# falcon-computing/falcon-genome

Hardware: AMD Instinct MI355X
Metric: PairHMM GCUPS + banded-SW GCUPS per GPU; end-to-end htc regions/sec at 8 GPUs (higher is better)
Workload: dtype fp32 (fp64 rescue)

## Files before the change

### falcon-genome_amd/csrc/phmm_cols.h

```cpp
#pragma once

namespace fcs {

constexpr int kColsClasses = 8;
constexpr int kColsMinR = 33;
__host__ __device__ constexpr int cols_C(int c) { return c == 0 ? 19 : 18 - c; }
__host__ __device__ constexpr int cols_hmax(int c) { return 16 * cols_C(c) - 1; }
__host__ __device__ inline int cols_class(int H) {
  for (int c = kColsClasses - 1; c >= 0; --c)
    if (H <= cols_hmax(c)) return c;
  return -1;
}
constexpr int kColsRing = 32;
constexpr int kColsChunks = 6;
constexpr int kColsChunkBytes = kColsRing * 4 * 16;
constexpr int kColsCapOff = kColsChunks * kColsChunkBytes;
constexpr int kColsTabOff = kColsCapOff + 4 * 8 * 8;
constexpr int kColsLds = kColsTabOff + 3 * 128 * 4;

__device__ __forceinline__ uint32_t vconst(uint32_t k) {
  uint32_t r;
  asm volatile("v_mov_b32 %0, %1" : "=v"(r) : "i"(k));
  return r;
}

struct ColsItem {
  float e1, e3, my, yy, mm, gm, mx, xx;
  uint32_t tlo, thi;
  float z;
};

__device__ __forceinline__ ColsItem cols_item(const PhmmTables<float>& tab, const RawRow& raw, int role, bool first,
                                              float ih) {
  ColsItem c;
  if (role == 2 || role == 3) {
    const RowP<float> q = row_params<float, false>(tab, raw);
    const float x0 = first ? ih * tab.dmatch[raw.gq & 127] : 1.f;
    const bool last = role == 3;
    c.e1 = q.e1 * x0;
    c.e3 = q.e3 * x0;
    c.my = last ? 0.f : q.my;
    c.yy = q.yy;
    c.mm = last ? 1.f : q.mm;
    c.gm = last ? 1.f : q.gm;
    c.mx = last ? 0.f : q.mx;
    c.xx = last ? 0.f : q.xx;
    const int bc = base_code((unsigned char)raw.rb);
    c.tlo = bc < 4 ? 1u << (8 * bc) : bc == 4 ? vconst(0x01010101u) : 0u;
    c.thi = 0x00000001u;
    c.z = 0.f;
  } else if (role == 4) {
    c.e1 = 1.f;
    c.e3 = 0.f;
    c.my = c.yy = c.mm = c.gm = 1.f;
    c.mx = c.xx = 0.f;
    c.tlo = vconst(0x01010101u);
    c.thi = vconst(0x00000101u);
    c.z = 0.f;
  } else {
    c.e1 = c.e3 = c.my = c.mm = c.gm = c.mx = c.xx = 0.f;
    c.yy = 1.f;
    c.tlo = c.thi = 0u;
    c.z = 1.f;
  }
  return c;
}

__device__ __forceinline__ void cols_put(unsigned char* smem, int slot, int seg, int h, const ColsItem& c) {
  float* const p = reinterpret_cast<float*>(smem + (seg * kColsRing + slot) * 16) + h;
  constexpr int F = kColsChunkBytes / 4;
  p[0] = c.e1;
  p[2] = c.e3;
  p[F] = c.my;
  p[F + 2] = c.yy;
  p[2 * F] = c.mm;
  p[2 * F + 2] = c.gm;
  p[3 * F] = c.mx;
  p[3 * F + 2] = c.xx;
  uint32_t* const q = reinterpret_cast<uint32_t*>(p);
  q[4 * F] = c.tlo;
  q[4 * F + 2] = c.thi;
  q[5 * F] = __float_as_uint(c.z);
  q[5 * F + 2] = __float_as_uint(c.z);
}

template <int NW>
__device__ __forceinline__ void cols_convert(const uint32_t (&raw)[NW + 1], int al, int i0, int H, uint32_t (&code)[NW],
                                             bool& other) {
#pragma unroll
  for (int d = 0; d < NW; ++d) {
    const uint32_t x = __builtin_amdgcn_alignbyte(raw[d + 1], raw[d], (uint32_t)al);
    const int rel = H - (i0 + 4 * d);
    const int nv = min(max(rel, 0), 4);
    const uint32_t vmask = nv >= 4 ? 0xFFFFFFFFu : (1u << (8 * nv)) - 1u;
    const uint32_t sel = (x >> 1) & vconst(0x07070707u);
    uint32_t c = __builtin_amdgcn_perm(vconst(0x04050505u), vconst(0x02030100u), sel);
    const uint32_t back = __builtin_amdgcn_perm(vconst(0x0000004Eu), vconst(0x54474341u), c);
    other |= ((back ^ x) & vmask) != 0u;
    c = (c & vmask) | (vconst(0x06060606u) & ~vmask);
    if (rel >= 0 && rel < 4) c = (c & ~(0xFFu << (8 * rel))) | (0x05u << (8 * rel));
    code[d] = c;
  }
}

template <int NW>
__device__ __forceinline__ void cols_load(const uint8_t* __restrict__ hb, int64_t ho, int H, int i0, uint32_t (&raw)[NW + 1],
                                          int& al) {
  const int64_t s = ho + i0;
  al = (int)(s & 3);
  const int64_t base = s - al;
  const uint32_t* const src = reinterpret_cast<const uint32_t*>(hb + base);
#pragma unroll
  for (int d = 0; d <= NW; ++d) raw[d] = (base + 4 * d < ho + H && H > 0) ? src[d] : 0u;
}

template <int C>
__global__ __launch_bounds__(64, 2) void phmm4_kernel(
    const PhmmDevBatch b, const int32_t* __restrict__ order, const int64_t* __restrict__ bounds, const int cls,
    const int K, const int tail_pairs, const PhmmTables<float> gtab, double* __restrict__ out,
    int32_t* __restrict__ rescue_list, unsigned long long* __restrict__ rescue_count, const float thr,
    const int use_rescue, int32_t* __restrict__ fb_list, unsigned long long* __restrict__ fb_count) {
  constexpr int NW = (C + 3) / 4;
  extern __shared__ __align__(16) unsigned char smem_raw[];
  const int lane = threadIdx.x;
  const int seg = lane >> 4;
  const int sl = lane & 15;
  const int sbase = lane & 48;
  const int th = sl >> 3, tk = sl & 7;
  const int i0 = sl * C;
  const int64_t cbeg = bounds[cls];
  const long long count = bounds[cls + 1] - cbeg;
  order += cbeg;
  PhmmTables<float> tab = gtab;
  {
    float* const t = reinterpret_cast<float*>(smem_raw + kColsTabOff);
    for (int i = lane; i < 128; i += 64) {
      t[i] = gtab.ph2pr[i];
      t[128 + i] = gtab.dmatch[i];
      t[256 + i] = gtab.dmis[i];
    }
    tab.ph2pr = t;
    tab.dmatch = t + 128;
    tab.dmis = t + 256;
  }
  const long long tailn = count < (long long)tail_pairs ? count : (long long)tail_pairs;
  const long long headn = count - tailn;
  const long long per = 8LL * K;
  const long long nb_head = (headn + per - 1) / per;
  const long long nbatch = nb_head + (tailn + 7) / 8;

  for (long long w = blockIdx.x; w < nbatch; w += gridDim.x) {
    const bool head = w < nb_head;
    const int Kb = head ? K : 1;
    const long long bstart = head ? w * per : headn + (w - nb_head) * 8;
    const long long bend = head ? min(headn, bstart + per) : min(count, bstart + 8);
    const long long idx = bstart + 2 * seg + th + 8LL * tk;
    const int pm = (tk < Kb && idx < bend) ? order[idx] : -1;
    int Rm = 0, Hm = 0;
    int64_t rom = 0, hom = 0;
    float Im = 0.f;
    if (pm >= 0) {
      const int ri = b.pair_read[pm], hi = b.pair_hap[pm];
      Rm = b.read_len[ri];
      Hm = b.hap_len[hi];
      rom = b.read_off[ri];
      hom = b.hap_off[hi];
      Im = tab.init_const / (float)Hm;
    }
    const int len = pm >= 0 ? Rm + 2 : 0;
    int incl = len;
#pragma unroll
    for (int d = 1; d < 8; d <<= 1) {
      const int v = __shfl_up(incl, d, 8);
      if (tk >= d) incl += v;
    }
    const int Gm = incl - len;
    const int totA = __builtin_amdgcn_ds_bpermute(4 * (sbase + 7), incl);
    const int totB = __builtin_amdgcn_ds_bpermute(4 * (sbase + 15), incl);
    const int nsteps = ((wave_max(max(totA, totB)) + 15) + 7) & ~7;
    int sb = sbase * 4;
    auto bp = [&](int v, int h, int k) {
      return __builtin_amdgcn_ds_bpermute(sb + 4 * (8 * h + min(k, 7)), v);
    };
    auto tG = [&](int h, int k) { return bp(Gm, h, k); };
    auto tR = [&](int h, int k) { return bp(Rm, h, k); };
    auto tH = [&](int h, int k) { return bp(Hm, h, k); };
    auto tP = [&](int h, int k) { return bp(pm, h, k); };
    auto tI = [&](int h, int k) { return __int_as_float(bp(__float_as_int(Im), h, k)); };
    auto t64 = [&](int64_t v, int h, int k) {
      const int lo = bp((int)v, h, k), hi = bp((int)(v >> 32), h, k);
      return (int64_t)(((uint64_t)(uint32_t)hi << 32) | (uint32_t)lo);
    };
    auto valid = [&](int h, int k) {
      const int pv = tP(h, k);
      return k < Kb && pv >= 0;
    };

    uint32_t cur[2][NW], nxt[2][NW];
    int nk[2], swr[2];
    unsigned other[2] = {0u, 0u};
    auto fetch_codes = [&](int h, int k, uint32_t (&dst)[NW]) {
      const bool ok = valid(h, k);
      const int Hk = tH(h, k);
      const int H = ok ? Hk : 0;
      const int64_t ho = t64(hom, h, k);
      uint32_t raw[NW + 1];
      int al;
      cols_load<NW>(b.hb, ok ? ho : 0, H, i0, raw, al);
      bool oth = false;
      cols_convert<NW>(raw, al, i0, H, dst, oth);
      const unsigned long long bal = __ballot(oth && ok);
      if (((bal >> sbase) & 0xFFFFull) != 0ull) other[h] |= 1u << k;
    };
#pragma unroll
    for (int h = 0; h < 2; ++h) {
#pragma unroll
      for (int d = 0; d < NW; ++d) cur[h][d] = 0x06060606u;
      fetch_codes(h, 0, nxt[h]);
      nk[h] = 0;
      swr[h] = valid(h, 0) ? tG(h, 0) : 0x3FFFFFFF;
    }
    int kc[2] = {0, 0};
    int cap[2], capp[2];
    auto load_cap = [&](int h) {
      const bool ok = valid(h, kc[h]);
      const int v = tG(h, kc[h]) + tR(h, kc[h]);
      cap[h] = ok ? v : -0x3FFFFFFF;
      capp[h] = tP(h, kc[h]);
    };
    load_cap(0);
    load_cap(1);

    int kp = 0;
    RawRow praw{-1, 0, 0, 0, 0, 0, 0};
    int prole = 0;
    float pih = 0.f;
    bool kok = false, nok = false;
    int kG = 0, kR = 0, nG = 0;
    float kI = 0.f;
    int64_t kro = 0;
    auto load_cursor = [&] {
      kok = valid(th, kp);
      kG = tG(th, kp);
      kR = tR(th, kp);
      kI = tI(th, kp);
      kro = t64(rom, th, kp);
      nok = valid(th, kp + 1);
      nG = tG(th, kp + 1);
    };
    load_cursor();
    auto stage_a = [&](int base) {
      const int g = base + tk;
      const bool adv = nok && g >= nG;
      if (__ballot(adv) != 0ull) {
        if (adv) ++kp;
        load_cursor();
      }
      const bool ok = kok;
      const int G = kG, R = kR;
      pih = kI;
      const int64_t ro = kro;
      const int r = g - G;
      int role = 0;
      if (ok && r >= 0 && r < R) role = r == R - 1 ? 3 : 2;
      else if (ok && r == R) role = 4;
      prole = role | (r == 0 ? 16 : 0);
      praw = (role == 2 || role == 3) ? load_raw(b, R, ro, r) : RawRow{-1, 0, 0, 0, 0, 0, 0};
    };
    auto stage_b = [&](int base) {
      cols_put(smem_raw, (base + tk) & (kColsRing - 1), seg, th,
               cols_item(tab, praw, prole & 15, (prole & 16) != 0, pih));
    };
    {
      ColsItem z = cols_item(tab, RawRow{-1, 0, 0, 0, 0, 0, 0}, 0, false, 0.f);
      cols_put(smem_raw, 16 + tk, seg, th, z);
      cols_put(smem_raw, 24 + tk, seg, th, z);
      stage_a(0);
      stage_b(0);
      stage_a(8);
    }

    pf2 Xn[C], In[C];
#pragma unroll
    for (int j = 0; j < C; ++j) {
      Xn[j] = pf2{1.f, 1.f};
      In[j] = pf2{0.f, 0.f};
    }
    pf2 dn = pf2{1.f, 1.f}, xo = pf2{1.f, 1.f}, xin = pf2{1.f, 1.f};
    const uint32_t segoff = (uint32_t)seg * (kColsRing * 16u) + lds_addr(smem_raw);

    for (int t0 = 0; t0 < nsteps; t0 += 8) {
      asm volatile("" : "+v"(sb));
#pragma unroll
      for (int h = 0; h < 2; ++h) {
        const bool ev = swr[h] + 16 <= t0 && nk[h] + 1 < Kb;
        if (__ballot(ev) != 0ull) {
          uint32_t tmp[NW];
          fetch_codes(h, nk[h] + 1, tmp);
          const bool vn = valid(h, nk[h] + 1);
          const int gn = tG(h, nk[h] + 1);
          if (ev) {
#pragma unroll
            for (int d = 0; d < NW; ++d) nxt[h][d] = tmp[d];
            ++nk[h];
            swr[h] = vn ? gn : 0x3FFFFFFF;
          }
        }
        if (swr[h] + 16 <= t0 && nk[h] + 1 >= Kb) swr[h] = 0x3FFFFFFF;
      }
      stage_b(t0 + 8);
      stage_a(t0 + 16);
#pragma unroll
      for (int h = 0; h < 2; ++h) {
        const bool adv = cap[h] >= 0 && cap[h] + 15 < t0;
        if (__ballot(adv) != 0ull) {
          if (adv) ++kc[h];
          load_cap(h);
        }
      }
      bool capo[2];
#pragma unroll
      for (int h = 0; h < 2; ++h) capo[h] = (other[h] >> kc[h]) & 1u;
      const int g0 = t0 - sl;
      const bool any_cap = __ballot(sl == 15 && ((unsigned)(cap[0] - g0) < 8u || (unsigned)(cap[1] - g0) < 8u)) != 0ull;
      unsigned swmask = 0u;
#pragma unroll
      for (int q = 0; q < 4; ++q)
#pragma unroll
        for (int h = 0; h < 2; ++h) {
          const int lo = __builtin_amdgcn_readlane(swr[h], 16 * q) - t0;
          if (lo < 8 && lo + 15 >= 0) {
            const int a = max(lo, 0), bnd = min(lo + 15, 7);
            swmask |= ((2u << bnd) - 1u) & ~((1u << a) - 1u);
          }
        }
      const uint32_t xs = (uint32_t)(g0 & (kColsRing - 1)) * 16u;
      const uint32_t capa = lds_addr(smem_raw) + kColsCapOff + seg * 64;

      auto step = [&](auto S_) {
        constexpr int S = decltype(S_)::value;
        const int g = g0 + S;
        if (swmask & (1u << S)) {
#pragma unroll
          for (int h = 0; h < 2; ++h) {
            const bool take = g == swr[h];
#pragma unroll
            for (int d = 0; d < NW; ++d) {
              uint32_t r;
              asm("v_cndmask_b32_e64 %0, %1, %2, %3" : "=v"(r) : "v"(cur[h][d]), "v"(nxt[h][d]), "s"(__ballot(take)));
              cur[h][d] = r;
            }
          }
        }
        asm volatile("" ::: "memory");
        const uint32_t pa = ((xs + (uint32_t)(S * 16)) & (uint32_t)((kColsRing - 1) * 16)) + segoff;
        typedef float f4 __attribute__((ext_vector_type(4)));
        typedef uint32_t u4 __attribute__((ext_vector_type(4)));
        auto ld4 = [&](int chunk) {
          return *reinterpret_cast<const __attribute__((address_space(3))) f4*>((uintptr_t)(pa + chunk * kColsChunkBytes));
        };
        const f4 r0 = ld4(0), r1 = ld4(1), r2 = ld4(2), r3 = ld4(3);
        const u4 cr = *reinterpret_cast<const __attribute__((address_space(3))) u4*>((uintptr_t)(pa + 4 * kColsChunkBytes));
        const pf2 z1 = *reinterpret_cast<const __attribute__((address_space(3))) pf2*>((uintptr_t)(pa + 5 * kColsChunkBytes));
        const pf2 z2 = *reinterpret_cast<const __attribute__((address_space(3))) pf2*>((uintptr_t)(pa + 5 * kColsChunkBytes + 8));
        const pf2 e1 = pf2{r0.x, r0.y}, e3 = pf2{r0.z, r0.w}, my = pf2{r1.x, r1.y}, yy = pf2{r1.z, r1.w};
        const pf2 mm = pf2{r2.x, r2.y}, gm = pf2{r2.z, r2.w}, mx = pf2{r3.x, r3.y}, xx = pf2{r3.z, r3.w};
        pf2 din, xnx;
        din.x = __int_as_float(__builtin_amdgcn_update_dpp(__float_as_int(z1.x), __float_as_int(dn.x), kDppRowShr1, 0xF, 0xF, false));
        din.y = __int_as_float(__builtin_amdgcn_update_dpp(__float_as_int(z1.y), __float_as_int(dn.y), kDppRowShr1, 0xF, 0xF, false));
        xnx.x = __int_as_float(__builtin_amdgcn_update_dpp(__float_as_int(z2.x), __float_as_int(xo.x), kDppRowShr1, 0xF, 0xF, false));
        xnx.y = __int_as_float(__builtin_amdgcn_update_dpp(__float_as_int(z2.y), __float_as_int(xo.y), kDppRowShr1, 0xF, 0xF, false));
        const pf2 xcur = xin;
        xin = xnx;
        uint32_t mA = 0, mB = 0;
        auto prior = [&](int j, const pf2 dep) {
          if ((j & 3) == 0) {
            mA = __builtin_amdgcn_perm(cr.z, cr.x, cur[0][j >> 2]);
            mB = __builtin_amdgcn_perm(cr.w, cr.y, cur[1][j >> 2]);
          }
          int a, c;
          asm volatile("v_bfe_i32 %0, %2, %3, 1\n\tv_bfe_i32 %1, %4, %3, 1"
                       : "=&v"(a), "=&v"(c)
                       : "v"(mA), "i"(8 * (j & 3)), "v"(mB), "v"(dep));
          return pf2{sel_v((uint32_t)a, e1.x, e3.x), sel_v((uint32_t)c, e1.y, e3.y)};
        };
        pf2 Mn = xcur * prior(0, xcur);
        pf2 D = din, Mp = pf2{0.f, 0.f}, Dp = pf2{0.f, 0.f};
#pragma unroll
        for (int j = 0; j < C; ++j) {
          const pf2 M = Mn;
          if (j > 0) D = __builtin_elementwise_fma(Mp, my, Dp * yy);
          pf2 I = In[j], Xo = Xn[j];
          asm volatile("" : "+v"(I), "+v"(Xo) : "v"(D));
          if (j + 1 < C) Mn = Xo * prior(j + 1, D);
          pf2 xn = __builtin_elementwise_fma(M, mm, __builtin_elementwise_fma(I, gm, D));
          pf2 in = __builtin_elementwise_fma(M, mx, I * xx);
          asm volatile("" : "+v"(xn), "+v"(in));
          Xn[j] = xn;
          In[j] = in;
          Mp = M;
          Dp = D;
        }
        dn = __builtin_elementwise_fma(Mp, my, Dp * yy);
        xo = Xn[C - 1];
        uint64_t keep;
        const uint32_t cpa = capa + 0u;
        const pf2 dnv = dn;
        asm volatile(
            "s_mov_b64 %0, exec\n\t"
            "s_mov_b64 exec, %3\n\t"
            "ds_write_b64 %1, %2 offset:%4\n\t"
            "s_mov_b64 exec, %0"
            : "=&s"(keep)
            : "v"(cpa), "v"(dnv), "s"(kTopLanes), "i"(8 * S)
            : "memory");
      };
      [&]<int... S>(std::integer_sequence<int, S...>) {
        (step(std::integral_constant<int, S>{}), ...);
      }(std::make_integer_sequence<int, 8>{});
      if (any_cap) {
#pragma unroll
        for (int h = 0; h < 2; ++h)
          if (sl == 15 && (unsigned)(cap[h] - g0) < 8u) {
            const pf2 v = *reinterpret_cast<const pf2*>(smem_raw + kColsCapOff + seg * 64 + 8 * (cap[h] - g0));
            const float acc = h ? v.y : v.x;
            const int p = capp[h];
            if (capo[h]) {
              const unsigned long long k = atomicAdd(fb_count, 1ull);
              fb_list[k] = p;
              out[p] = __builtin_nan("");
            } else if (use_rescue && acc < thr) {
              const unsigned long long k = atomicAdd(rescue_count, 1ull);
              rescue_list[k] = p;
              out[p] = __builtin_nan("");
            } else {
              out[p] = (double)(log10f(acc) - tab.log10_init);
            }
          }
      }
    }
  }
}

}
```

### falcon-genome_amd/csrc/phmm_kernels.hip

```cpp
#include <hip/hip_runtime.h>

#include <algorithm>
#include <cstdlib>

#include <utility>

#include "fcship_internal.h"

namespace fcs {

constexpr int PFD = 2;
template <typename T> struct alignas(2 * sizeof(T)) PhRing {
  T X, I;
};

__device__ __forceinline__ float fma_t(float a, float b, float c) { return fmaf(a, b, c); }
__device__ __forceinline__ double fma_t(double a, double b, double c) { return fma(a, b, c); }

__device__ __forceinline__ unsigned char base_code(unsigned char b) {
  return b == 'A' ? 0 : b == 'C' ? 1 : b == 'G' ? 2 : b == 'T' ? 3 : b == 'N' ? 4 : 5;
}
__device__ __forceinline__ int base_mask(int rb) {
  const int c = base_code((unsigned char)rb);
  return c == 4 ? 0x7F : c == 5 ? 0x10 : (1 << c) | 0x10;
}
__device__ __forceinline__ float sel_bits(uint32_t m, float a, float b) {
  return __uint_as_float((__float_as_uint(a) & m) | (__float_as_uint(b) & ~m));
}
__device__ __forceinline__ double sel_bits(uint32_t m, double a, double b) {
  const unsigned long long mm = ((unsigned long long)m << 32) | m;
  return __longlong_as_double((long long)(((unsigned long long)__double_as_longlong(a) & mm) |
                                          ((unsigned long long)__double_as_longlong(b) & ~mm)));
}

template <typename T, int W>
__device__ __forceinline__ T dpp_shr1(T old, T src) {
  if constexpr (W == 16) {
    return dpp_row_shr1<T>(old, src);
  } else {
    static_assert(W == 64, "segments are 16 or 64 lanes");
    if constexpr (sizeof(T) == 4) {
      return __int_as_float(dpp_wave_shr1_i(__float_as_int(old), __float_as_int(src)));
    } else {
      const long long o = __double_as_longlong(old), v = __double_as_longlong(src);
      const int lo = dpp_wave_shr1_i((int)o, (int)v);
      const int hi = dpp_wave_shr1_i((int)(o >> 32), (int)(v >> 32));
      return __longlong_as_double(((long long)hi << 32) | (unsigned int)lo);
    }
  }
}

__device__ __forceinline__ void acc_add(float& a, float x) { asm("v_add_f32 %0, %1, %2" : "=v"(a) : "v"(a), "v"(x)); }
__device__ __forceinline__ void acc_add(double& a, double x) {
  asm("v_add_f64 %0, %1, %2" : "=v"(a) : "v"(a), "v"(x));
}

template <typename T>
struct RowP {
  T e1, e3, my, yy;
  T mm, gm, mx, xx;
  int rbase;
  int rmask;
};

template <typename T>
struct LaneState {
  T Mo, Do;
  T Xp;
  T Xo, Io;
};

template <typename T, bool EXACT, bool SUM, bool BC, bool COND, int W, int S>
__device__ __forceinline__ void phmm_step(LaneState<T>& L, PhRing<T> (&pf)[PFD], int (&hq)[PFD],
                                          const unsigned char* __restrict__ hapl, const RowP<T>& p,
                                          PhRing<T>* __restrict__ ring, const int t0, const int sl, const bool top,
                                          const int lim, T& accM, T& accI) {
  const int t = t0 + S;
  const PhRing<T> cur = pf[0];
  const int hb = hq[0];
#pragma unroll
  for (int k = 0; k + 1 < PFD; ++k) {
    pf[k] = pf[k + 1];
    hq[k] = hq[k + 1];
  }
  pf[PFD - 1] = ring[t + W + PFD];
  hq[PFD - 1] = hapl[t + W + PFD - sl];
  const T Xu = dpp_shr1<T, W>(cur.X, L.Xo);
  const T I = dpp_shr1<T, W>(cur.I, L.Io);
  T prior;
  if constexpr (BC) {
    prior = (hb == p.rbase || hb == 'N') ? p.e1 : p.e3;
  } else {
    prior = sel_bits((uint32_t)__builtin_amdgcn_sbfe(p.rmask, hb, 1), p.e1, p.e3);
  }
  const T M = L.Xp * prior;
  T D, Xn, In;
  if constexpr (EXACT) {
    D = L.Mo * p.my + L.Do * p.yy;
    Xn = (M * p.mm + I * p.gm) + D * p.gm;
    In = M * p.mx + I * p.xx;
  } else {
    D = fma_t(L.Mo, p.my, L.Do * p.yy);
    Xn = fma_t(M, p.mm, fma_t(I, p.gm, D));
    In = fma_t(M, p.mx, I * p.xx);
  }
  if (top) {
    PhRing<T> o;
    o.X = Xn;
    o.I = In;
    ring[t + 1] = o;
  }
  if constexpr (SUM) {
    if constexpr (!COND) {
      acc_add(accI, I);
    } else {
      if (t <= lim) acc_add(accI, I);
      if (t == lim) accM = D + M;
    }
  }
  L.Xp = Xu;
  L.Xo = Xn;
  L.Io = In;
  L.Mo = M;
  L.Do = D;
}

template <typename T, bool EXACT, bool SUM, bool BC, bool COND, int W>
__device__ __forceinline__ void phmm_block(LaneState<T>& L, PhRing<T> (&pf)[PFD], int (&hq)[PFD],
                                           const unsigned char* __restrict__ hapl, const RowP<T>& p,
                                           PhRing<T>* __restrict__ ring, const int t0, const int sl, const bool top,
                                           const int lim, T& accM, T& accI) {
  [&]<int... S>(std::integer_sequence<int, S...>) {
    (phmm_step<T, EXACT, SUM, BC, COND, W, S>(L, pf, hq, hapl, p, ring, t0, sl, top, lim, accM, accI), ...);
  }(std::make_integer_sequence<int, 16>{});
}

struct RawRow {
  int rb, bq, dq, gq;
  int niq, ndq, ngq;
};

__device__ __forceinline__ RawRow load_raw(const PhmmDevBatch& b, int R, int64_t ro, int pos) {
  RawRow r{-1, 0, 0, 0, 0, 0, 0};
  if (pos < R) {
    const int64_t a = ro + pos;
    r.rb = b.rb[a];
    r.bq = b.bq[a];
    r.dq = b.dq[a];
    r.gq = b.gq[a];
    if (pos + 1 < R) {
      r.niq = b.iq[a + 1];
      r.ndq = b.dq[a + 1];
      r.ngq = b.gq[a + 1];
    }
  }
  return r;
}

template <typename T, bool EXACT>
__device__ __forceinline__ RowP<T> row_params(const PhmmTables<T>& tab, const RawRow& r) {
  RowP<T> p;
  p.e1 = p.e3 = p.my = p.yy = p.mm = p.gm = p.mx = p.xx = (T)0;
  p.rbase = -1;
  p.rmask = -1;
  if (r.rb < 0) return p;
  const int q = r.bq & 127, qd = r.dq & 127, qc = r.gq & 127;
  p.rbase = r.rb;
  p.rmask = base_mask(r.rb);
  p.e1 = tab.dmatch[q];
  p.e3 = (r.rb == 'N') ? p.e1 : tab.dmis[q];
  p.my = tab.ph2pr[qd];
  p.yy = tab.ph2pr[qc];
  const int ni = r.niq & 127, nd = r.ndq & 127, nc = r.ngq & 127;
  const int hi = ni > nd ? ni : nd, lo = ni > nd ? nd : ni;
  p.mm = tab.mm[((hi * (hi + 1)) >> 1) + lo];
  p.gm = tab.dmatch[nc];
  p.mx = tab.ph2pr[ni];
  p.xx = tab.ph2pr[nc];
  if constexpr (!EXACT) p.my = p.my * p.gm;
  return p;
}

template <typename T, bool EXACT, bool SUM, bool BC, int W>
__device__ __forceinline__ void phmm_stripe(const RowP<T>& p, PhRing<T>* __restrict__ ring,
                                            const unsigned char* __restrict__ hapl, const int sl, const int nblk,
                                            const int lim, const int ulim, T& accM, T& accI,
                                            const PhmmTables<T>& tab, const RawRow& nraw, RowP<T>& np,
                                            const bool top) {
  LaneState<T> L;
  L.Mo = L.Do = L.Xp = L.Xo = L.Io = (T)0;
  PhRing<T> pf[PFD];
  int hq[PFD];
#pragma unroll
  for (int k = 0; k < PFD; ++k) {
    pf[k] = ring[W + k];
    hq[k] = hapl[W + k - sl];
  }
  if (!SUM || 15 < ulim)
    phmm_block<T, EXACT, SUM, BC, false, W>(L, pf, hq, hapl, p, ring, 0, sl, top, lim, accM, accI);
  else
    phmm_block<T, EXACT, SUM, BC, true, W>(L, pf, hq, hapl, p, ring, 0, sl, top, lim, accM, accI);
  np = row_params<T, EXACT>(tab, nraw);
  for (int blk = 1; blk < nblk; ++blk) {
    if (!SUM || 16 * blk + 15 < ulim)
      phmm_block<T, EXACT, SUM, BC, false, W>(L, pf, hq, hapl, p, ring, 16 * blk, sl, top, lim, accM, accI);
    else
      phmm_block<T, EXACT, SUM, BC, true, W>(L, pf, hq, hapl, p, ring, 16 * blk, sl, top, lim, accM, accI);
  }
}

template <typename T>
__host__ __device__ constexpr int ring_stride(int nslot) {
  return nslot * (int)sizeof(PhRing<T>);
}

template <typename T, bool EXACT, bool RESCUE_PASS, int W = 16>
__global__ __launch_bounds__(64, (sizeof(T) == 4 && !EXACT) ? 4 : 1) void phmm_kernel(const PhmmDevBatch b, const int32_t* __restrict__ order,
                                                  const unsigned long long* __restrict__ count_dev,
                                                  long long count_host, const int64_t* __restrict__ bounds,
                                                  const int cls, const int nslot, const PhmmTables<T> tab,
                                                  double* __restrict__ out, int32_t* __restrict__ rescue_list,
                                                  unsigned long long* __restrict__ rescue_count, const float thr,
                                                  const int use_rescue, const int nseg) {
  extern __shared__ __align__(16) unsigned char smem_raw[];
  const int lane = threadIdx.x;
  const int seg = lane / W;
  const int sl = lane & (W - 1);
  const bool own_seg = seg < nseg;
  const int rseg = own_seg ? seg : 0;
  PhRing<T>* const ring = reinterpret_cast<PhRing<T>*>(smem_raw + rseg * ring_stride<T>(nslot));
  unsigned char* const hapl = smem_raw + (size_t)nseg * ring_stride<T>(nslot) + rseg * nslot;
  const bool top = own_seg && sl == W - 1;
  long long count = count_dev ? (long long)(*count_dev) : count_host;
  if (bounds) {
    order += bounds[cls];
    count = bounds[cls + 1] - bounds[cls];
  }
  const long long ngroups = (count + nseg - 1) / nseg;

  for (long long g = blockIdx.x; g < ngroups; g += gridDim.x) {
    const long long idx = g * nseg + seg;
    const int p = (own_seg && idx < count) ? order[idx] : -1;
    int R = 0, H = 0;
    int64_t ro = 0, ho = 0;
    if (p >= 0) {
      const int ri = b.pair_read[p], hi = b.pair_hap[p];
      R = b.read_len[ri];
      H = b.hap_len[hi];
      ro = b.read_off[ri];
      ho = b.hap_off[hi];
    }
    const bool active = (p >= 0) && R > 0 && H > 0;
    if (p >= 0 && !active && sl == 0) out[p] = -INFINITY;
    const int nstr = active ? (R + W - 1) / W : 0;
    const int Hmax = wave_max(active ? H : 0);
    const int nstr_max = wave_max(nstr);
    if (nstr_max == 0) continue;

    const T init = active ? tab.init_const / (T)H : (T)0;
    const T x0 = active ? init * tab.dmatch[b.gq[ro] & 127] : (T)0;
    __syncthreads();
    bool other = false;
    constexpr int kHB = 8;
    for (int s0 = sl; s0 < nslot; s0 += W * kHB) {
      unsigned char raw[kHB];
#pragma unroll
      for (int u = 0; u < kHB; ++u) {
        const int c = s0 + W * u - W;
        raw[u] = (active && c >= 1 && c <= H && c + W < nslot) ? b.hb[ho + c - 1] : (unsigned char)0;
      }
#pragma unroll
      for (int u = 0; u < kHB; ++u) {
        const int s = s0 + W * u, c = s - W;
        if (own_seg && s < nslot) {
          PhRing<T> v;
          v.X = (c >= 0 && c <= H) ? x0 : (T)0;
          v.I = 0;
          ring[s] = v;
          const bool in = active && c >= 1 && c <= H;
          const unsigned char code = in ? base_code(raw[u]) : (unsigned char)6;
          other |= code == 5;
          hapl[s] = code;
        }
      }
    }
    const bool bytecmp = __ballot(other) != 0ull;
    if (bytecmp && own_seg)
      for (int s = sl; s < nslot; s += W) {
        const int c = s - W;
        hapl[s] = (active && c >= 1 && c <= H) ? b.hb[ho + c - 1] : (unsigned char)0;
      }
    __syncthreads();

    RowP<T> prm = row_params<T, EXACT>(tab, load_raw(b, active ? R : 0, ro, sl));
    T accM = 0, accI = 0;
    const int sum_stripe = active ? (R - 1) / W : -1;
    const int sum_lane = active ? (R - 1) % W : -1;
    for (int st = 0; st < nstr_max; ++st) {
      const RawRow nraw = load_raw(b, active ? R : 0, ro, (st + 1) * W + sl);
      RowP<T> nprm;
      const bool seg_sums = (st == sum_stripe);
      const int any_sum = wave_max(seg_sums ? 1 : 0);
      if (any_sum) {
        const int cont = wave_max((active && nstr > st + 1) ? 1 : 0);
        const int lim = (seg_sums && sl == sum_lane) ? sl + H : -1;
        const int ulim = -wave_max((seg_sums && sl == sum_lane) ? -(sl + H) : -0x7FFFFFFF);
        accM = accI = 0;
        const int tend = cont ? Hmax + W - 1 : wave_max(seg_sums ? sum_lane + H : 0);
        RowP<T> sp = prm;
        if (lim >= 0) sp.my = sp.yy = (T)1;
        if (bytecmp)
          phmm_stripe<T, EXACT, true, true, W>(sp, ring, hapl, sl, (tend + 16) >> 4, lim, ulim, accM, accI, tab, nraw, nprm, top);
        else
          phmm_stripe<T, EXACT, true, false, W>(sp, ring, hapl, sl, (tend + 16) >> 4, lim, ulim, accM, accI, tab, nraw, nprm, top);
        if (seg_sums && sl == sum_lane) {
          const T sum = accM + accI;
          if constexpr (RESCUE_PASS) {
            out[p] = log10(sum) - (double)tab.log10_init;
          } else {
            if (use_rescue && sum < (T)thr) {
              const unsigned long long k = atomicAdd(rescue_count, 1ull);
              rescue_list[k] = p;
              out[p] = __builtin_nan("");
            } else {
              out[p] = (double)(log10f((float)sum) - (float)tab.log10_init);
            }
          }
        }
      } else {
        if (bytecmp)
          phmm_stripe<T, EXACT, false, true, W>(prm, ring, hapl, sl, (Hmax + W + 15) >> 4, -1, -1, accM, accI, tab, nraw, nprm, top);
        else
          phmm_stripe<T, EXACT, false, false, W>(prm, ring, hapl, sl, (Hmax + W + 15) >> 4, -1, -1, accM, accI, tab, nraw, nprm, top);
      }
      prm = nprm;
    }
  }
}

}

#include "phmm2.h"
#include "phmm_stream.h"
#include "phmm_cols.h"

namespace fcs {

static __host__ __device__ int nslot_for(int max_hap_len) { return ((max_hap_len + 51 + 15) / 16) * 16; }
static __host__ __device__ int nslot_for_w(int max_hap_len, int W) {
  return ((max_hap_len + 2 * W + 19 + 15) / 16) * 16;
}

static_assert(kPhmmLaunchClasses <= 16 && kPhmmKeyClassShift + 4 <= kPhmmKeyBits, "class fits the key");
__host__ __device__ inline int phmm_class(int H) {
  const int c = (nslot_for(H) - 224 + 31) / 32;
  return c < 0 ? 0 : c > kPhmmClasses - 1 ? kPhmmClasses - 1 : c;
}

__host__ __device__ inline int phmm_launch_class(int R, int H, int& stream_cls) {
  stream_cls = -1;
  if (R >= kStreamMinR && R <= kStreamMaxR && H >= 1) {
    static_assert(kColsMinR <= kStreamMinR, "column-blocked streams take every streamed read");
    const int cc = cols_class(H);
    stream_cls = cc >= 0 ? 0 : stream_class(H);
    if (cc >= 0) return kLongClasses + cc;
    if (stream_cls >= 2) return kStreamClasses - 1 - stream_cls;
    stream_cls = -1;
  }
  return kLongClasses + kColsLaunch + kPhmmClasses - 1 - phmm_class(max(H, 0));
}

__device__ __forceinline__ uint32_t phmm_key(const PhmmDevBatch& b, long long p) {
  const int R = b.read_len[b.pair_read[p]];
  const int H = b.hap_len[b.pair_hap[p]];
  int sc;
  const uint32_t cf = (uint32_t)phmm_launch_class(R, H, sc);
  const uint32_t hh = 0xFFFu - (uint32_t)min(max(H, 0), 0xFFF);
  uint32_t low;
  if (sc >= 0)
    low = hh;
  else
    low = ((3u - (uint32_t)min((max(R, 0) + 15) >> 4, 3)) << 10) | (0x3FFu - (uint32_t)min(max(H, 0) >> 2, 0x3FF));
  return (cf << kPhmmKeyClassShift) | low;
}

constexpr int kPhmmBins = 1 << (kPhmmKeyBits - 4);
constexpr int kBinBlock = 1024, kBinItems = 4;
__device__ __forceinline__ int phmm_bin(const PhmmDevBatch& b, long long p) { return (int)(phmm_key(b, p) >> 4); }

__global__ __launch_bounds__(kBinBlock) void phmm_bin_count_kernel(const PhmmDevBatch b, uint32_t* __restrict__ hist,
                                                                    unsigned long long* __restrict__ counters) {
  __shared__ uint32_t h[kPhmmBins];
  for (int i = threadIdx.x; i < kPhmmBins; i += kBinBlock) h[i] = 0;
  if (blockIdx.x == 0 && threadIdx.x == 0) {
    counters[0] = 0ull;
    counters[1] = 0ull;
  }
  __syncthreads();
  const long long base = (long long)blockIdx.x * (kBinBlock * kBinItems);
  for (int k = 0; k < kBinItems; ++k) {
    const long long p = base + (long long)k * kBinBlock + threadIdx.x;
    if (p < b.n_pairs) atomicAdd(&h[phmm_bin(b, p)], 1u);
  }
  __syncthreads();
  for (int i = threadIdx.x; i < kPhmmBins; i += kBinBlock)
    if (h[i]) atomicAdd(&hist[i], h[i]);
}

__global__ __launch_bounds__(kBinBlock) void phmm_bin_scan_kernel(uint32_t* __restrict__ hist,
                                                                   uint32_t* __restrict__ cursor, long long n,
                                                                   int64_t* __restrict__ bounds) {
  constexpr int kPer = kPhmmBins / kBinBlock;
  __shared__ uint32_t part[kBinBlock];
  const int t = threadIdx.x;
  uint32_t v[kPer], sum = 0;
  for (int j = 0; j < kPer; ++j) {
    v[j] = hist[t * kPer + j];
    sum += v[j];
  }
  part[t] = sum;
  __syncthreads();
  for (int off = 1; off < kBinBlock; off <<= 1) {
    const uint32_t x = t >= off ? part[t - off] : 0u;
    __syncthreads();
    part[t] += x;
    __syncthreads();
  }
  uint32_t run = part[t] - sum;
  for (int j = 0; j < kPer; ++j) {
    const int bin = t * kPer + j;
    cursor[bin] = run;
    if ((bin & 255) == 0 && (bin >> 8) < kPhmmLaunchClasses) bounds[bin >> 8] = run;
    run += v[j];
    hist[bin] = 0u;
  }
  if (t == 0) bounds[kPhmmLaunchClasses] = n;
}

__global__ __launch_bounds__(kBinBlock) void phmm_bin_scatter_kernel(const PhmmDevBatch b,
                                                                      uint32_t* __restrict__ cursor,
                                                                      int32_t* __restrict__ idx) {
  __shared__ uint32_t cnt[kPhmmBins], at[kPhmmBins];
  for (int i = threadIdx.x; i < kPhmmBins; i += kBinBlock) cnt[i] = 0;
  __syncthreads();
  const long long base = (long long)blockIdx.x * (kBinBlock * kBinItems);
  int bin[kBinItems];
  uint32_t rank[kBinItems];
  for (int k = 0; k < kBinItems; ++k) {
    const long long p = base + (long long)k * kBinBlock + threadIdx.x;
    bin[k] = p < b.n_pairs ? phmm_bin(b, p) : -1;
    rank[k] = bin[k] >= 0 ? atomicAdd(&cnt[bin[k]], 1u) : 0u;
  }
  __syncthreads();
  for (int i = threadIdx.x; i < kPhmmBins; i += kBinBlock)
    if (cnt[i]) at[i] = atomicAdd(&cursor[i], cnt[i]);
  __syncthreads();
  for (int k = 0; k < kBinItems; ++k)
    if (bin[k] >= 0) idx[at[bin[k]] + rank[k]] = (int32_t)(base + (long long)k * kBinBlock + threadIdx.x);
}

int launch_phmm_bin_schedule(const PhmmDevBatch& b, int32_t* idx_out, int64_t* bounds, unsigned long long* counters,
                             uint32_t* hist, uint32_t* cursor, hipStream_t s) {
  static_assert(kPhmmBins % kBinBlock == 0 && (kPhmmLaunchClasses << 8) <= kPhmmBins, "bins");
  const long long n = b.n_pairs > 0 ? b.n_pairs : 0;
  const unsigned nb = (unsigned)std::max<long long>((n + kBinBlock * kBinItems - 1) / (kBinBlock * kBinItems), 1);
  hipLaunchKernelGGL(phmm_bin_count_kernel, dim3(nb), dim3(kBinBlock), 0, s, b, hist, counters);
  FCS_HIP_CHECK(hipGetLastError());
  hipLaunchKernelGGL(phmm_bin_scan_kernel, dim3(1), dim3(kBinBlock), 0, s, hist, cursor, n, bounds);
  FCS_HIP_CHECK(hipGetLastError());
  if (n > 0) {
    hipLaunchKernelGGL(phmm_bin_scatter_kernel, dim3(nb), dim3(kBinBlock), 0, s, b, cursor, idx_out);
    FCS_HIP_CHECK(hipGetLastError());
  }
  return FCS_OK;
}

constexpr size_t kLdsBytes = 160 * 1024;

template <typename T, bool EXACT, bool RESCUE, int W = 16>
static int launch_one(const PhmmDevBatch& b, const int32_t* order, const unsigned long long* count_dev,
                      long long count_host, const int64_t* bounds, int cls, int nslot, long long max_groups,
                      const PhmmTables<T>& tab, double* out, int32_t* rescue_list, unsigned long long* rescue_count,
                      float thr, bool use_rescue, hipStream_t s) {
  int nseg = 64 / W;
  size_t lds = (size_t)nseg * (ring_stride<T>(nslot) + nslot);
  if (lds > kLdsBytes && nseg > 1) {
    nseg = 1;
    lds = (size_t)ring_stride<T>(nslot) + nslot;
    max_groups *= 4;
  }
  if (lds > kLdsBytes)
    return fail(FCS_ERR_UNSUPPORTED, "[E::fcship] haplotype too long for the LDS boundary ring (max_hap_len " +
                                         std::to_string(nslot - 67) + ")");
  auto kern = phmm_kernel<T, EXACT, RESCUE, W>;
  if (lds > 64 * 1024)
    FCS_HIP_CHECK(hipFuncSetAttribute((const void*)kern, hipFuncAttributeMaxDynamicSharedMemorySize, (int)lds));
  long long grid = max_groups;
  const long long cap = 65536;
  if (grid > cap) grid = cap;
  if (grid < 1) grid = 1;
  hipLaunchKernelGGL(kern, dim3((unsigned)grid), dim3(64), lds, s, b, order, count_dev, count_host, bounds, cls, nslot,
                     tab, out, rescue_list, rescue_count, thr, use_rescue ? 1 : 0, nseg);
  FCS_HIP_CHECK(hipGetLastError());
  return FCS_OK;
}

static int stream_pairs_per_segment(int64_t n) {
  static const int forced = [] {
    const char* e = std::getenv("FCSHIP_STREAM_K");
    return e ? std::atoi(e) : 0;
  }();
  if (forced > 0) return std::min(forced, kStreamMaxK);
  const int64_t k = n / (4 * 24576);
  return (int)std::max<int64_t>(1, std::min<int64_t>(kStreamMaxK, k));
}

static int cols_pairs_per_half(int64_t n) {
  static const int forced = [] {
    const char* e = std::getenv("FCSHIP_STREAM_K");
    return e ? std::atoi(e) : 0;
  }();
  if (forced > 0) return std::min(forced, 8);
  const int64_t k = n / (8 * 24576);
  return (int)std::max<int64_t>(1, std::min<int64_t>(8, k));
}

int launch_phmm_forward(const PhmmDevBatch& b, const int32_t* order, int64_t count, int max_hap_len,
                        const int64_t* bounds, const DeviceTables& t, bool exact, double* out, int32_t* rescue_list,
                        unsigned long long* rescue_count, float thr, bool use_rescue, int32_t* fb_list,
                        unsigned long long* fb_count, hipStream_t s) {
  if (count <= 0) return FCS_OK;
  const long long groups = (count + 3) / 4;
  const int ns_max = nslot_for(max_hap_len);
  const int c_max = phmm_class(max_hap_len);
  hipStream_t fs[kForkStreams];
  if (const int rc = fork_streams(s, fs); rc != FCS_OK) return rc;
  int fork = 0;
  for (int j = 0; j < kLongClasses; ++j) {
    const int sc = kStreamClasses - 1 - j;
    const int lo = j == 0 ? stream_class_hmax(sc - 1) : cols_hmax(0);
    if (max_hap_len <= lo) continue;
    const int hmax = std::min(stream_class_hmax(sc), max_hap_len);
    hipStream_t st = fs[fork++ % kForkStreams];
    if (exact) {
      const int rc = launch_one<float, true, false>(b, order, nullptr, count, bounds, j, nslot_for(hmax), groups, t.tf,
                                                   out, rescue_list, rescue_count, thr, use_rescue, st);
      if (rc != FCS_OK) return rc;
      continue;
    }
    const size_t lds = (size_t)stream_lds(hmax);
    if (lds > kLdsBytes) return fail(FCS_ERR_UNSUPPORTED, "[E::fcship] streamed PairHMM class exceeds LDS");
    const int K = stream_pairs_per_segment(count);
    const int w = stream_class_waves(sc);
    const int tail = 2 * 4 * 1024 * w;
    const unsigned grid = (unsigned)std::min<long long>(
        std::max<long long>((count + 4 * K - 1) / (4 * K) + (tail + 3) / 4, 1), 65536);
    auto launch = [&](auto kern) -> int {
      if (lds > 64 * 1024)
        FCS_HIP_CHECK(hipFuncSetAttribute((const void*)kern, hipFuncAttributeMaxDynamicSharedMemorySize, (int)lds));
      hipLaunchKernelGGL(kern, dim3(grid), dim3(64), lds, st, b, order, bounds, j, K, tail, stream_nslot(hmax),
                         stream_hstride(hmax), t.tf, out, rescue_list, rescue_count, thr, use_rescue ? 1 : 0, fb_list,
                         fb_count);
      FCS_HIP_CHECK(hipGetLastError());
      return FCS_OK;
    };
    const int rc = w >= 3 ? launch(phmm3_kernel<3>) : w == 2 ? launch(phmm3_kernel<2>) : launch(phmm3_kernel<1>);
    if (rc != FCS_OK) return rc;
  }
  for (int c = 0; c < kColsLaunch; ++c) {
    const int lo = c + 1 < kColsLaunch ? cols_hmax(c + 1) : 0;
    if (max_hap_len <= lo) continue;
    const int j = kLongClasses + c;
    hipStream_t st = fs[fork++ % kForkStreams];
    if (exact) {
      const int rc = launch_one<float, true, false>(b, order, nullptr, count, bounds, j,
                                                   nslot_for(std::min(cols_hmax(c), max_hap_len)), groups, t.tf, out,
                                                   rescue_list, rescue_count, thr, use_rescue, st);
      if (rc != FCS_OK) return rc;
      continue;
    }
    const int K = cols_pairs_per_half(count);
    const int tail = 1024 * 3 * 8;
    const unsigned grid = (unsigned)std::min<long long>(
        std::max<long long>((count + 8 * K - 1) / (8 * K) + (tail + 7) / 8, 1), 65536);
    auto launch = [&](auto kern) -> int {
      hipLaunchKernelGGL(kern, dim3(grid), dim3(64), (size_t)kColsLds, st, b, order, bounds, j, K, tail, t.tf, out,
                         rescue_list, rescue_count, thr, use_rescue ? 1 : 0, fb_list, fb_count);
      FCS_HIP_CHECK(hipGetLastError());
      return FCS_OK;
    };
    static_assert(cols_C(0) == 19 && cols_C(1) == 17 && cols_C(7) == 11 && kColsClasses == 8, "launch table below");
    int rc;
    switch (cols_C(c)) {
      case 19: rc = launch(phmm4_kernel<19>); break;
      case 17: rc = launch(phmm4_kernel<17>); break;
      case 16: rc = launch(phmm4_kernel<16>); break;
      case 15: rc = launch(phmm4_kernel<15>); break;
      case 14: rc = launch(phmm4_kernel<14>); break;
      case 13: rc = launch(phmm4_kernel<13>); break;
      case 12: rc = launch(phmm4_kernel<12>); break;
      default: rc = launch(phmm4_kernel<11>); break;
    }
    if (rc != FCS_OK) return rc;
  }
  constexpr long long kGroupedGrid = 8192;
  int gfork = 0;
  for (int j = kPhmmClasses - 1 - c_max; j < kPhmmClasses; ++j) {
    const int c = kPhmmClasses - 1 - j;
    const int lc = kLongClasses + kColsLaunch + j;
    const int ns = (c == kPhmmClasses - 1) ? ns_max : std::min(224 + 32 * c, ns_max);
    hipStream_t st = fs[1 + gfork++ % (kForkStreams - 1)];
    const int ns2 = ns + 16;
    const size_t lds2 = (size_t)phmm2_lds(ns2);
    if (!exact && lds2 <= kLdsBytes) {
      if (lds2 > 64 * 1024)
        FCS_HIP_CHECK(
            hipFuncSetAttribute((const void*)phmm2_kernel, hipFuncAttributeMaxDynamicSharedMemorySize, (int)lds2));
      const unsigned grid = (unsigned)std::min<long long>(std::max<long long>(groups, 1), kGroupedGrid);
      hipLaunchKernelGGL(phmm2_kernel, dim3(grid), dim3(64), lds2, st, b, order, bounds, lc, ns2, t.tf, out,
                         rescue_list, rescue_count, thr, use_rescue ? 1 : 0);
      FCS_HIP_CHECK(hipGetLastError());
      continue;
    }
    const int rc = exact ? launch_one<float, true, false>(b, order, nullptr, count, bounds, lc, ns, groups, t.tf, out,
                                                           rescue_list, rescue_count, thr, use_rescue, st)
                         : launch_one<float, false, false>(b, order, nullptr, count, bounds, lc, ns, groups, t.tf, out,
                                                            rescue_list, rescue_count, thr, use_rescue, st);
    if (rc != FCS_OK) return rc;
  }
  if (const int rc = join_streams(s, fs); rc != FCS_OK) return rc;
  if (exact) return FCS_OK;
  return launch_one<float, false, false>(b, fb_list, fb_count, 0, nullptr, 0, ns_max,
                                         std::min<long long>(groups, 2048), t.tf, out, rescue_list, rescue_count, thr,
                                         use_rescue, s);
}

int launch_phmm_rescue(const PhmmDevBatch& b, const int32_t* list, const unsigned long long* count_dev,
                       int64_t max_count, int max_hap_len, const DeviceTables& t, bool exact, double* out,
                       hipStream_t s) {
  if (max_count <= 0) return FCS_OK;
  const int ns64 = nslot_for_w(max_hap_len, 64);
  if ((size_t)ring_stride<double>(ns64) + ns64 <= kLdsBytes) {
    const long long g64 = std::min<long long>(max_count, 4096);
    if (exact)
      return launch_one<double, true, true, 64>(b, list, count_dev, 0, nullptr, 0, ns64, g64, t.td, out, nullptr,
                                                nullptr, 0.f, false, s);
    return launch_one<double, false, true, 64>(b, list, count_dev, 0, nullptr, 0, ns64, g64, t.td, out, nullptr,
                                               nullptr, 0.f, false, s);
  }
  long long groups = (max_count + 3) / 4;
  if (groups > 2048) groups = 2048;
  if (exact)
    return launch_one<double, true, true>(b, list, count_dev, 0, nullptr, 0, nslot_for(max_hap_len), groups, t.td, out,
                                          nullptr, nullptr, 0.f, false, s);
  return launch_one<double, false, true>(b, list, count_dev, 0, nullptr, 0, nslot_for(max_hap_len), groups, t.td, out,
                                         nullptr, nullptr, 0.f, false, s);
}

}
```

Baseline: 3982.

## Add single-pair-per-segment cols PairHMM kernel and make it default

Adds phmm5_kernel, a column-tiled PairHMM forward variant in which each 16-lane segment processes one pair stream in fp32 scalar form instead of packed halves. It uses a 48-slot LDS ring of pf2 chunks, up to 16 pairs per stream, and a smaller LDS footprint sized to allow more waves per CU. The launcher now routes every cols class to the new kernel by default, with an FCSHIP_COLS env override to return to the packed path. The cost is lower per-lane packing density, which is traded against simpler scheduling and higher occupancy.

```diff
diff --git a/falcon-genome_amd/csrc/phmm_cols.h b/falcon-genome_amd/csrc/phmm_cols.h
--- a/falcon-genome_amd/csrc/phmm_cols.h
+++ b/falcon-genome_amd/csrc/phmm_cols.h
@@ -442,4 +442,325 @@
   }
 }
 
-}
+constexpr int kCols1Ring = 48;
+constexpr int kCols1Chunks = 5;
+constexpr int kCols1ChunkBytes = kCols1Ring * 4 * 8;
+constexpr int kCols1CapOff = kCols1Chunks * kCols1ChunkBytes;
+constexpr int kCols1TabOff = kCols1CapOff + 4 * 16 * 4;
+constexpr int kCols1Lds = kCols1TabOff + 3 * 128 * 4;
+constexpr int kCols1MaxK = 16;
+__host__ __device__ constexpr int cols1_waves(int C) { return 3; }
+static_assert(kCols1Lds <= 10240, "16 waves per CU");
+
+typedef uint32_t pu2 __attribute__((ext_vector_type(2)));
+
+__device__ __forceinline__ void cols1_put(unsigned char* smem, int slot, int seg, const ColsItem& c) {
+  unsigned char* const p = smem + (seg * kCols1Ring + slot) * 8;
+  *reinterpret_cast<pf2*>(p) = pf2{c.e1, c.e3};
+  *reinterpret_cast<pf2*>(p + kCols1ChunkBytes) = pf2{c.my, c.yy};
+  *reinterpret_cast<pf2*>(p + 2 * kCols1ChunkBytes) = pf2{c.mm, c.gm};
+  *reinterpret_cast<pf2*>(p + 3 * kCols1ChunkBytes) = pf2{c.mx, c.xx};
+  *reinterpret_cast<pu2*>(p + 4 * kCols1ChunkBytes) = pu2{c.tlo, c.thi | (c.z != 0.f ? 0x01000000u : 0u)};
+}
+
+template <int C>
+__global__ __launch_bounds__(64, cols1_waves(C)) void phmm5_kernel(
+    const PhmmDevBatch b, const int32_t* __restrict__ order, const int64_t* __restrict__ bounds, const int cls,
+    const int K, const int tail_pairs, const PhmmTables<float> gtab, double* __restrict__ out,
+    int32_t* __restrict__ rescue_list, unsigned long long* __restrict__ rescue_count, const float thr,
+    const int use_rescue, int32_t* __restrict__ fb_list, unsigned long long* __restrict__ fb_count) {
+  constexpr int NW = (C + 3) / 4;
+  extern __shared__ __align__(16) unsigned char smem_raw[];
+  const int lane = threadIdx.x;
+  const int seg = lane >> 4;
+  const int sl = lane & 15;
+  const int sbase = lane & 48;
+  const int i0 = sl * C;
+  const int64_t cbeg = bounds[cls];
+  const long long count = bounds[cls + 1] - cbeg;
+  order += cbeg;
+  PhmmTables<float> tab = gtab;
+  {
+    float* const t = reinterpret_cast<float*>(smem_raw + kCols1TabOff);
+    for (int i = lane; i < 128; i += 64) {
+      t[i] = gtab.ph2pr[i];
+      t[128 + i] = gtab.dmatch[i];
+      t[256 + i] = gtab.dmis[i];
+    }
+    tab.ph2pr = t;
+    tab.dmatch = t + 128;
+    tab.dmis = t + 256;
+  }
+  const long long tailn = count < (long long)tail_pairs ? count : (long long)tail_pairs;
+  const long long headn = count - tailn;
+  const long long per = 4LL * K;
+  const long long nb_head = (headn + per - 1) / per;
+  const long long nbatch = nb_head + (tailn + 3) / 4;
+
+  for (long long w = blockIdx.x; w < nbatch; w += gridDim.x) {
+    const bool head = w < nb_head;
+    const int Kb = head ? K : 1;
+    const long long bstart = head ? w * per : headn + (w - nb_head) * 4;
+    const long long bend = head ? min(headn, bstart + per) : min(count, bstart + 4);
+    const long long idx = bstart + seg + 4LL * sl;
+    const int pm = (sl < Kb && idx < bend) ? order[idx] : -1;
+    int Rm = 0, Hm = 0;
+    int64_t rom = 0, hom = 0;
+    float Im = 0.f;
+    if (pm >= 0) {
+      const int ri = b.pair_read[pm], hi = b.pair_hap[pm];
+      Rm = b.read_len[ri];
+      Hm = b.hap_len[hi];
+      rom = b.read_off[ri];
+      hom = b.hap_off[hi];
+      Im = tab.init_const / (float)Hm;
+    }
+    const int len = pm >= 0 ? Rm + 2 : 0;
+    int incl = len;
+#pragma unroll
+    for (int d = 1; d < 16; d <<= 1) {
+      const int v = __shfl_up(incl, d, 16);
+      if (sl >= d) incl += v;
+    }
+    const int Gm = incl - len;
+    const int tot = __builtin_amdgcn_ds_bpermute(4 * (sbase + 15), incl);
+    const int nsteps = ((wave_max(tot) + 15) + 15) & ~15;
+    int sb = sbase * 4;
+    auto bp = [&](int v, int k) { return __builtin_amdgcn_ds_bpermute(sb + 4 * min(k, 15), v); };
+    auto tG = [&](int k) { return bp(Gm, k); };
+    auto tR = [&](int k) { return bp(Rm, k); };
+    auto tH = [&](int k) { return bp(Hm, k); };
+    auto tP = [&](int k) { return bp(pm, k); };
+    auto tI = [&](int k) { return __int_as_float(bp(__float_as_int(Im), k)); };
+    auto t64 = [&](int64_t v, int k) {
+      const int lo = bp((int)v, k), hi = bp((int)(v >> 32), k);
+      return (int64_t)(((uint64_t)(uint32_t)hi << 32) | (uint32_t)lo);
+    };
+    auto valid = [&](int k) {
+      const int pv = tP(k);
+      return k < Kb && pv >= 0;
+    };
+
+    uint32_t cur[NW], nxt[NW];
+    int nk, swr;
+    unsigned other = 0u;
+    auto fetch_codes = [&](int k, uint32_t (&dst)[NW]) {
+      const bool ok = valid(k);
+      const int Hk = tH(k);
+      const int H = ok ? Hk : 0;
+      const int64_t ho = t64(hom, k);
+      uint32_t raw[NW + 1];
+      int al;
+      cols_load<NW>(b.hb, ok ? ho : 0, H, i0, raw, al);
+      bool oth = false;
+      cols_convert<NW>(raw, al, i0, H, dst, oth);
+      const unsigned long long bal = __ballot(oth && ok);
+      if (((bal >> sbase) & 0xFFFFull) != 0ull) other |= 1u << k;
+    };
+#pragma unroll
+    for (int d = 0; d < NW; ++d) cur[d] = 0x06060606u;
+    fetch_codes(0, nxt);
+    nk = 0;
+    swr = valid(0) ? tG(0) : 0x3FFFFFFF;
+    int kc = 0, cap, capp;
+    auto load_cap = [&] {
+      const bool ok = valid(kc);
+      const int v = tG(kc) + tR(kc);
+      cap = ok ? v : -0x3FFFFFFF;
+      capp = tP(kc);
+    };
+    load_cap();
+
+    int kp = 0;
+    RawRow praw{-1, 0, 0, 0, 0, 0, 0};
+    int prole = 0;
+    float pih = 0.f;
+    bool kok = false, nok = false;
+    int kG = 0, kR = 0, nG = 0;
+    float kI = 0.f;
+    int64_t kro = 0;
+    auto load_cursor = [&] {
+      kok = valid(kp);
+      kG = tG(kp);
+      kR = tR(kp);
+      kI = tI(kp);
+      kro = t64(rom, kp);
+      nok = valid(kp + 1);
+      nG = tG(kp + 1);
+    };
+    load_cursor();
+    auto stage_a = [&](int base) {
+      const int g = base + sl;
+      const bool adv = nok && g >= nG;
+      if (__ballot(adv) != 0ull) {
+        if (adv) ++kp;
+        load_cursor();
+      }
+      const int r = g - kG;
+      int role = 0;
+      if (kok && r >= 0 && r < kR) role = r == kR - 1 ? 3 : 2;
+      else if (kok && r == kR) role = 4;
+      pih = kI;
+      prole = role | (r == 0 ? 16 : 0);
+      praw = (role == 2 || role == 3) ? load_raw(b, kR, kro, r) : RawRow{-1, 0, 0, 0, 0, 0, 0};
+    };
+    auto stage_b = [&](int base) {
+      cols1_put(smem_raw, (int)((unsigned)(base + sl) % (unsigned)kCols1Ring), seg,
+                cols_item(tab, praw, prole & 15, (prole & 16) != 0, pih));
+    };
+    {
+      cols1_put(smem_raw, 32 + sl, seg, cols_item(tab, RawRow{-1, 0, 0, 0, 0, 0, 0}, 0, false, 0.f));
+      stage_a(0);
+      stage_b(0);
+      stage_a(16);
+    }
+
+    float Xn[C], In[C];
+#pragma unroll
+    for (int j = 0; j < C; ++j) {
+      Xn[j] = 1.f;
+      In[j] = 0.f;
+    }
+    float dn = 1.f, xo = 1.f, xin = 1.f;
+    const uint32_t segoff = (uint32_t)seg * (kCols1Ring * 8u) + lds_addr(smem_raw);
+
+    for (int t0 = 0; t0 < nsteps; t0 += 16) {
+      asm volatile("" : "+v"(sb));
+      {
+        const bool ev = swr + 16 <= t0 && nk + 1 < Kb;
+        if (__ballot(ev) != 0ull) {
+          uint32_t tmp[NW];
+          fetch_codes(nk + 1, tmp);
+          const bool vn = valid(nk + 1);
+          const int gn = tG(nk + 1);
+          if (ev) {
+#pragma unroll
+            for (int d = 0; d < NW; ++d) nxt[d] = tmp[d];
+            ++nk;
+            swr = vn ? gn : 0x3FFFFFFF;
+          }
+        }
+        if (swr + 16 <= t0 && nk + 1 >= Kb) swr = 0x3FFFFFFF;
+      }
+      stage_b(t0 + 16);
+      stage_a(t0 + 32);
+      {
+        const bool adv = cap >= 0 && cap + 15 < t0;
+        if (__ballot(adv) != 0ull) {
+          if (adv) ++kc;
+          load_cap();
+        }
+      }
+      const bool capo = (other >> kc) & 1u;
+      const int gb = t0 - sl;
+      const bool any_cap = __ballot(sl == 15 && (unsigned)(cap - gb) < 16u) != 0ull;
+      unsigned swmask = 0u;
+#pragma unroll
+      for (int q = 0; q < 4; ++q) {
+        const int lo = __builtin_amdgcn_readlane(swr, 16 * q) - t0;
+        if (lo < 16 && lo + 15 >= 0) {
+          const int a = max(lo, 0), bnd = min(lo + 15, 15);
+          swmask |= ((2u << bnd) - 1u) & ~((1u << a) - 1u);
+        }
+      }
+      uint32_t xs = ((uint32_t)(gb + kCols1Ring) % (uint32_t)kCols1Ring) * 8u;
+      uint32_t capa = lds_addr(smem_raw) + kCols1CapOff + seg * 64;
+      int g0 = gb;
+
+#pragma nounroll
+      for (int pass = 0; pass < 2; ++pass) {
+        auto step = [&](auto S_) {
+          constexpr int S = decltype(S_)::value;
+          const int g = g0 + S;
+          if (swmask & (1u << S)) {
+            const bool take = g == swr;
+#pragma unroll
+            for (int d = 0; d < NW; ++d) {
+              uint32_t r;
+              asm("v_cndmask_b32_e64 %0, %1, %2, %3" : "=v"(r) : "v"(cur[d]), "v"(nxt[d]), "s"(__ballot(take)));
+              cur[d] = r;
+            }
+          }
+          asm volatile("" ::: "memory");
+          const uint32_t a0 = xs + (uint32_t)(S * 8);
+          const uint32_t pa = min(a0, a0 - (uint32_t)(kCols1Ring * 8)) + segoff;
+          auto ld2 = [&](int chunk) {
+            return *reinterpret_cast<const __attribute__((address_space(3))) pf2*>((uintptr_t)(pa + chunk * kCols1ChunkBytes));
+          };
+          const pf2 r0 = ld2(0), r1 = ld2(1), r2 = ld2(2), r3 = ld2(3);
+          const pu2 cr = *reinterpret_cast<const __attribute__((address_space(3))) pu2*>((uintptr_t)(pa + 4 * kCols1ChunkBytes));
+          const float e1 = r0.x, e3 = r0.y, my = r1.x, yy = r1.y, mm = r2.x, gm = r2.y, mx = r3.x, xx = r3.y;
+          const float z = (float)(cr.y >> 24);
+          const float din = __int_as_float(__builtin_amdgcn_update_dpp(__float_as_int(z), __float_as_int(dn), kDppRowShr1, 0xF, 0xF, false));
+          const float xnx = __int_as_float(__builtin_amdgcn_update_dpp(__float_as_int(z), __float_as_int(xo), kDppRowShr1, 0xF, 0xF, false));
+          const float xcur = xin;
+          xin = xnx;
+          uint32_t mA = 0;
+          auto prior = [&](int j, const float dep) {
+            if ((j & 3) == 0) mA = __builtin_amdgcn_perm(cr.y, cr.x, cur[j >> 2]);
+            int a;
+            asm volatile("v_bfe_i32 %0, %1, %2, 1" : "=v"(a) : "v"(mA), "i"(8 * (j & 3)), "v"(dep));
+            return sel_v((uint32_t)a, e1, e3);
+          };
+          float Mn = xcur * prior(0, xcur);
+          float D = din, Mp = 0.f, Dp = 0.f;
+#pragma unroll
+          for (int j = 0; j < C; ++j) {
+            const float M = Mn;
+            if (j > 0) D = __builtin_fmaf(Mp, my, Dp * yy);
+            float I = In[j], Xo = Xn[j];
+            asm volatile("" : "+v"(I), "+v"(Xo) : "v"(D));
+            if (j + 1 < C) Mn = Xo * prior(j + 1, D);
+            float xn = __builtin_fmaf(M, mm, __builtin_fmaf(I, gm, D));
+            float in = __builtin_fmaf(M, mx, I * xx);
+            asm volatile("" : "+v"(xn), "+v"(in));
+            Xn[j] = xn;
+            In[j] = in;
+            Mp = M;
+            Dp = D;
+          }
+          dn = __builtin_fmaf(Mp, my, Dp * yy);
+          xo = Xn[C - 1];
+          uint64_t keep;
+          const uint32_t cpa = capa + 0u;
+          const float dnv = dn;
+          asm volatile(
+              "s_mov_b64 %0, exec\n\t"
+              "s_mov_b64 exec, %3\n\t"
+              "ds_write_b32 %1, %2 offset:%4\n\t"
+              "s_mov_b64 exec, %0"
+              : "=&s"(keep)
+              : "v"(cpa), "v"(dnv), "s"(kTopLanes), "i"(4 * S)
+              : "memory");
+        };
+        [&]<int... S>(std::integer_sequence<int, S...>) {
+          (step(std::integral_constant<int, S>{}), ...);
+        }(std::make_integer_sequence<int, 8>{});
+        g0 += 8;
+        swmask >>= 8;
+        capa += 32;
+        xs += 64;
+        xs = min(xs, xs - (uint32_t)(kCols1Ring * 8));
+      }
+      if (any_cap) {
+        if (sl == 15 && (unsigned)(cap - gb) < 16u) {
+          const float acc = *reinterpret_cast<const float*>(smem_raw + kCols1CapOff + seg * 64 + 4 * (cap - gb));
+          const int p = capp;
+          if (capo) {
+            const unsigned long long k = atomicAdd(fb_count, 1ull);
+            fb_list[k] = p;
+            out[p] = __builtin_nan("");
+          } else if (use_rescue && acc < thr) {
+            const unsigned long long k = atomicAdd(rescue_count, 1ull);
+            rescue_list[k] = p;
+            out[p] = __builtin_nan("");
+          } else {
+            out[p] = (double)(log10f(acc) - tab.log10_init);
+          }
+        }
+      }
+    }
+  }
+}
+
+}
diff --git a/falcon-genome_amd/csrc/phmm_kernels.hip b/falcon-genome_amd/csrc/phmm_kernels.hip
--- a/falcon-genome_amd/csrc/phmm_kernels.hip
+++ b/falcon-genome_amd/csrc/phmm_kernels.hip
@@ -2,6 +2,7 @@
 
 #include <algorithm>
 #include <cstdlib>
+#include <cstring>
 
 #include <utility>
 
@@ -525,6 +526,30 @@
   return (int)std::max<int64_t>(1, std::min<int64_t>(8, k));
 }
 
+static int cols1_forced_k() {
+  static const int forced = [] {
+    const char* e = std::getenv("FCSHIP_STREAM_K");
+    return e ? std::atoi(e) : 0;
+  }();
+  return forced > 0 ? std::min(forced, kCols1MaxK) : 0;
+}
+static int cols1_pairs_per_stream(int64_t n) {
+  if (const int f = cols1_forced_k()) return f;
+  const int64_t k = n / (4 * 32768);
+  return (int)std::max<int64_t>(1, std::min<int64_t>(kCols1MaxK, k));
+}
+
+static bool cols_single(int c) {
+  static const int forced = [] {
+    const char* e = std::getenv("FCSHIP_COLS");
+    if (!e) return 0;
+    return !std::strcmp(e, "single") ? 1 : !std::strcmp(e, "packed") ? 2 : 0;
+  }();
+  if (forced) return forced == 1;
+  static constexpr bool kSingle[kColsClasses] = {true, true, true, true, true, true, true, true};
+  return kSingle[c];
+}
+
 int launch_phmm_forward(const PhmmDevBatch& b, const int32_t* order, int64_t count, int max_hap_len,
                         const int64_t* bounds, const DeviceTables& t, bool exact, double* out, int32_t* rescue_list,
                         unsigned long long* rescue_count, float thr, bool use_rescue, int32_t* fb_list,
@@ -579,6 +604,32 @@
       if (rc != FCS_OK) return rc;
       continue;
     }
+    if (cols_single(c)) {
+      const int K = cols1_pairs_per_stream(count);
+      const int tail = cols1_forced_k() ? 4 : 1024 * cols1_waves(cols_C(c)) * 4;
+      const unsigned grid = (unsigned)std::min<long long>(
+          std::max<long long>((count + 4 * K - 1) / (4 * K) + (tail + 3) / 4, 1), 65536);
+      auto launch = [&](auto kern) -> int {
+        hipLaunchKernelGGL(kern, dim3(grid), dim3(64), (size_t)kCols1Lds, st, b, order, bounds, j, K, tail, t.tf, out,
+                           rescue_list, rescue_count, thr, use_rescue ? 1 : 0, fb_list, fb_count);
+        FCS_HIP_CHECK(hipGetLastError());
+        return FCS_OK;
+      };
+      static_assert(cols_C(0) == 19 && cols_C(1) == 17 && cols_C(7) == 11 && kColsClasses == 8, "launch table below");
+      int rc;
+      switch (cols_C(c)) {
+        case 19: rc = launch(phmm5_kernel<19>); break;
+        case 17: rc = launch(phmm5_kernel<17>); break;
+        case 16: rc = launch(phmm5_kernel<16>); break;
+        case 15: rc = launch(phmm5_kernel<15>); break;
+        case 14: rc = launch(phmm5_kernel<14>); break;
+        case 13: rc = launch(phmm5_kernel<13>); break;
+        case 12: rc = launch(phmm5_kernel<12>); break;
+        default: rc = launch(phmm5_kernel<11>); break;
+      }
+      if (rc != FCS_OK) return rc;
+      continue;
+    }
     const int K = cols_pairs_per_half(count);
     const int tail = 1024 * 3 * 8;
     const unsigned grid = (unsigned)std::min<long long>(
```

Result: faster. 4459, median of 6 (+12.0%).
